# lucasgattas/ComfyUI-Egregora-Audio-Super-Resolution

Measured on AMD Instinct MI355X. Metric: audio-sec/sec (xRT) FlashSR 48kHz + Fat-Llama 800-iter at 1/2/4/8 MI355X, higher is better.
Workload: dtype f32(f16x2); 1 GPU; chain60: per GPU 60 s stereo 48 kHz; FlashSR (5.12 s chunks, hop 4.62 s, student_ldm 1-step + VAE + sr_vocoder, declared architecture, synthetic weights, chunk-sharded with one all-gather, WOLA) then Fat-Llama max_iterations=800 thr=0.6 normalize on autoscale off, threshold reading of the HEADLINE value: 'default' (SPEC.md section 3 default = absolute level on int16-scale samples, hard threshold, ; arch=gfx950:sramecc+:xnack-, chunks=13, rows_per_pass=32

## Files before the change

### comfyui-egregora-audio-super-resolution_amd/csrc/egr_flashsr.cpp

```cpp
#include <math.h>
#include <cmath>
#include <stdio.h>
#include <stdlib.h>
#include <string.h>

#include <atomic>
#include <chrono>
#include <map>
#include <memory>
#include <mutex>
#include <new>
#include <string>
#include <unordered_map>
#include <vector>

#include "egr_common.h"

extern "C" {
int egr_pack_weight(const float* src, float* dst, int layout, int K, int N, int Ci, int Co, int KH, int KW, void* stream);
int egr_phase_weights(const float* w_oihw, float* dst4, int Co, int Ci, void* stream);
int egr_winograd_pack_u(const float* w_oihw, float* dst, const double* G_dev, int np, int Co, int Ci, void* stream);
}

namespace {
// ... 964 lines not shown
            OKR(conv3(m, t, h, "vae.encoder.down." + std::to_string(lv) + ".downsample.conv", 2, 0, ACT_NONE, nullptr, 0));
            h = std::move(t);
        }
    }
    OKR(vae_res(m, t, h, "vae.encoder.mid.block_1")); h = std::move(t);
    OKR(vae_attn(m, t, h, "vae.encoder.mid.attn_1")); h = std::move(t);
    OKR(vae_res(m, t, h, "vae.encoder.mid.block_2")); h = std::move(t);
    OKR(groupnorm(m, t, h, "vae.encoder.norm_out", 1e-6f, true));
    OKR(conv3(m, h, t, "vae.encoder.conv_out"));
    Ten mom;
    OKR(conv1x1(m, mom, h, "vae.quant_conv"));
    const int64_t rows = mom.d[0] * mom.d[1] * mom.d[2];
    OKR(new_ten(m, z, {mom.d[0], mom.d[1], mom.d[2], c.z_ch}));
    EGR_HIP(hipMemcpy2DAsync(z.p, (size_t)c.z_ch * 4, mom.p, (size_t)2 * c.z_ch * 4, (size_t)c.z_ch * 4, (size_t)rows, hipMemcpyDeviceToDevice, m->st));
    return EGR_OK;
}

int vae_decode(M* m, Ten& y, const Ten& z) {
    const egr_flashsr_config& c = m->cfg;
    Ten h, t;
    m->next_out_ra = true;
    OKR(conv1x1(m, t, z, "vae.post_quant_conv"));
    OKR(conv3(m, h, t, "vae.decoder.conv_in"));
    OKR(vae_res(m, t, h, "vae.decoder.mid.block_1")); h = std::move(t);
    OKR(vae_attn(m, t, h, "vae.decoder.mid.attn_1")); h = std::move(t);
    OKR(vae_res(m, t, h, "vae.decoder.mid.block_2")); h = std::move(t);
    for (int lv = c.vae_levels - 1; lv >= 0; --lv) {
        for (int b = 0; b <= c.vae_res; ++b) {
            OKR(vae_res(m, t, h, "vae.decoder.up." + std::to_string(lv) + ".block." + std::to_string(b)));
            h = std::move(t);
        }
        if (lv != 0) {
            OKR(conv3(m, t, h, "vae.decoder.up." + std::to_string(lv) + ".upsample.conv", 1, 1));
            h = std::move(t);
        }
    }
    OKR(groupnorm(m, t, h, "vae.decoder.norm_out", 1e-6f, true));
    return conv3(m, y, t, "vae.decoder.conv_out");
}

int unet_block(M* m, Ten& y, const Ten& x, const std::string& base, bool has_attn) {
    const egr_flashsr_config& c = m->cfg;
    Ten h, sc, r;
    OKR(gn_conv3(m, h, x, base + ".res.in_norm", 1e-5f, base + ".res.in_conv", nullptr, m->ptr(base + ".res.in_conv.bias_t")));
    const float* scp = x.p;
    if (m->has(base + ".res.skip.weight")) { OKR(conv1x1(m, sc, x, base + ".res.skip")); scp = sc.p; }
    OKR(gn_conv3(m, r, h, base + ".res.out_norm", 1e-5f, base + ".res.out_conv", scp));
    h.release(); sc.release();
    if (!has_attn) { y = std::move(r); return EGR_OK; }
    const int B = (int)r.d[0], H = (int)r.d[1], W = (int)r.d[2], Cc = (int)r.d[3];
    const int T = H * W, heads = Cc / c.head_dim;
    Ten g0, t;
    OKR(groupnorm(m, g0, r, base + ".st.norm", 1e-6f, false));
    OKR(conv1x1(m, t, g0, base + ".st.proj_in"));
    g0.release();
    t.view({(int64_t)B * T, Cc});
    for (int a = 1; a <= 2; ++a) {
        const std::string an = base + ".st.attn" + std::to_string(a);
        Ten n_, q, k, v, o, t2;
        OKR(layernorm(m, n_, t, an + "_ln"));
        m->next_out_ra = true;
        OKR(linear(m, q, n_, an + ".to_q", nullptr, ACT_NONE, false));
        m->next_out_ra = true;
        OKR(linear(m, k, n_, an + ".to_k", nullptr, ACT_NONE, false));
        m->next_out_ra = true;
        OKR(linear(m, v, n_, an + ".to_v", nullptr, ACT_NONE, false));
        OKR(attention(m, o, q, k, v, B, T, Cc, heads));
        OKR(linear(m, t2, o, an + ".to_out", t.p));
        t = std::move(t2);
    }
    Ten ln, u, g, t3;
    OKR(layernorm(m, ln, t, base + ".st.ff_ln"));
    OKR(linear(m, u, ln, base + ".st.ff.geglu"));
    OKR(new_ten(m, g, {(int64_t)B * T, 4 * Cc}));
    {
        float* ra = nullptr;
        if (B == m->R) OKR(rs_for_output(m, g, &ra));
        if (ra) OKR(egr_geglu_ra(u.p, g.p, (int64_t)B * T, 4 * Cc, m->R, ra, m->st));
        else OKR(egr_geglu(u.p, g.p, (int64_t)B * T, 4 * Cc, m->st));
    }
    m->next_out_ra = true;
    OKR(linear(m, t3, g, base + ".st.ff.out", t.p));
    t3.view({B, H, W, Cc});
    m->next_out_ra = true;
    return conv1x1(m, y, t3, base + ".st.proj_out", r.p);
}

int unet(M* m, Ten& out, Ten&& x0) {
    std::vector<Ten> skips;
    Ten h = std::move(x0), t;
    for (size_t i = 0; i < m->blk_name.size(); ++i) {
        const std::string& name = m->blk_name[i];
        const std::string base = "unet." + name;
        const std::string part = name.substr(0, name.find('.'));
        const std::string kind = name.substr(name.rfind('.') + 1);
        if (kind == "conv_in") {
            OKR(conv3(m, t, h, base));
            Ten cp = t.alias();
            skips.push_back(std::move(t));
            h = std::move(cp);
        } else if (kind == "down") {
            m->next_out_ra = true;
            OKR(conv3(m, t, h, base + ".conv", 2, 0, ACT_NONE, nullptr, 1));
            Ten cp = t.alias();
            skips.push_back(std::move(t));
            h = std::move(cp);
        } else if (kind == "up") {
            OKR(conv3(m, t, h, base + ".conv", 1, 1));
            h = std::move(t);
        } else {
            if (part == "out") {
                Ten cat;
                OKR(concat(m, cat, h, skips.back()));
                skips.pop_back();
                h = std::move(cat);
            }
            OKR(unet_block(m, t, h, base, m->blk_attn[i] != 0));
            if (part == "in") {
                Ten cp = t.alias();
                skips.push_back(std::move(t));
                h = std::move(cp);
            } else {
                h = std::move(t);
            }
        }
    }
    OKR(groupnorm(m, t, h, "unet.out_norm", 1e-5f, true));
    return conv3(m, out, t, "unet.out_conv");
}

int amp(M* m, Ten& y, Ten&& h, int j) {
    const egr_flashsr_config& c = m->cfg;
    Ten acc;
    for (int ki = 0; ki < c.voc_n_kernels; ++ki) {
        const int k = c.voc_kernels[ki];
        Ten x;
        const Ten* cur = &h;
        for (int di = 0; di < c.voc_n_dils; ++di) {
            const int d = c.voc_dils[di];
            const std::string b = "voc.amp." + std::to_string(j) + "." + std::to_string(ki) + "." + std::to_string(di);
            Ten xt, xc, xs, xn;
            {
                const Wt* w1 = m->get(b + ".conv1.weight");
                const Wt* w2 = m->get(b + ".conv2.weight");
                const int Cc = (int)cur->d[2];
                if (m->fused_amp && m->h2 && m->h2_mode == 1 && w1 && w2 && w1->w2 && w2->w2 && Cc == 16 && w1->Cout == Cc && w2->Cout == Cc && (k & 1) &&
                    k <= 11 && d * (k - 1) / 2 <= 25 && c.aa_taps == 12 && cur->d[1] >= 16) {
                    OKR(new_ten(m, xn, {cur->d[0], cur->d[1], cur->d[2]}));
                    ProfScope ps(m);
                    OKR(egr_amp_unit_h2(cur->p, xn.p, (int)cur->d[0], (int)cur->d[1], Cc, k, d, m->ptr(b + ".alpha1"), m->ptr(b + ".beta1"), w1->w2, w1->w_scale,
                                        m->ptr(b + ".conv1.bias"), m->ptr(b + ".alpha2"), m->ptr(b + ".beta2"), w2->w2, w2->w_scale, m->ptr(b + ".conv2.bias"),
                                        m->filt, c.aa_taps, m->st));
                    const double fl = 2.0 * 2.0 * (double)cur->d[0] * cur->d[1] * Cc * Cc * k;
                    if (ps.on) ps.end(Cc == 16 ? "k_amp_unit<16>" : "k_amp_unit<32>", fl, b);
                    if (m->count_flops) m->flops += fl;
                    x = std::move(xn);
                    cur = &x;
                    continue;
                }
            }
            OKR(snake(m, xt, *cur, b + ".alpha1", b + ".beta1"));
            OKR(conv1d(m, xc, xt, b + ".conv1", k, 1, d, d * (k - 1) / 2));
            xt.release();
            OKR(snake(m, xs, xc, b + ".alpha2", b + ".beta2"));
            xc.release();
            OKR(conv1d(m, xn, xs, b + ".conv2", k, 1, 1, (k - 1) / 2, ACT_NONE, cur->p));
            x = std::move(xn);
            cur = &x;
        }
        if (ki == 0) {
            acc = std::move(x);
        } else if (ki + 1 < c.voc_n_kernels) {
            Ten s;
            OKR(eltwise(m, s, acc, x.p, EW_ADD));
            acc = std::move(s);
        } else {
            return eltwise(m, y, acc, x.p, EW_ADD_SCALE, 1.0f / c.voc_n_kernels, 0.f, true);
        }
    }
    return eltwise(m, y, acc, nullptr, EW_SCALE, 1.0f / c.voc_n_kernels, 0.f, true);
}

int vocoder(M* m, Ten& y, const Ten& mel_hat, const float* wave, int B) {
    const egr_flashsr_config& c = m->cfg;
    const int T = (int)mel_hat.d[1], Fm = (int)mel_hat.d[2];
    const int n = c.voc_n_rates;
    std::vector<Ten> feats(n);
    {
        Ten e0;
        e0.view({B, c.chunk, 1});
        e0.p = const_cast<float*>(wave);
        const Ten* e = &e0;
        for (int i = 0; i < n; ++i) {
            const int r = c.voc_rates[n - 1 - i];
            m->next_out_ra = i + 1 < n;
            OKR(conv1d(m, feats[i], *e, "voc.wave_enc." + std::to_string(i), 2 * r + 1, r, 1, r, ACT_LEAKY));
            e = &feats[i];
        }
    }
    Ten mh;
    mh.view({B, T, Fm});
    mh.p = mel_hat.p;
    Ten h;
    m->next_out_ra = true;
    OKR(conv1d(m, h, mh, "voc.conv_pre", 7, 1, 1, 3, ACT_NONE, feats[n - 1].p));
    feats[n - 1].release();
    for (int j = 0; j < n; ++j) {
        const int r = c.voc_rates[j];
        const int kt = up_kernel(r);
        const int Bc = (int)h.d[0], Lin = (int)h.d[1], Ci = (int)h.d[2];
        const Wt* wt = m->get("voc.ups." + std::to_string(j) + ".weight");
        const int Co = wt->Cout / kt;
        Ten Y, out, hx;
        hx.view({(int64_t)Bc * Lin, 1, 1, Ci});
        hx.p = h.p;
        hx.rs = h.rs;
        OKR(conv(m, Y, hx, "voc.ups." + std::to_string(j), Bc * Lin, 1, 1, Ci, 1, 1, kt * Co, 1, 1, 1, 1, 0, 0, 0, ACT_NONE, false, nullptr, nullptr, 0.f, wt));
        OKR(new_ten(m, out, {Bc, (int64_t)Lin * r, Co}));
        const float* add = (j <= n - 2) ? feats[n - 2 - j].p : nullptr;
        OKR(egr_col2im_convtr1d(Y.p, m->ptr("voc.ups." + std::to_string(j) + ".bias"), add, out.p, Bc, Lin, Lin * r, Co, kt, r, (kt - r) / 2, m->st));
        Y.release();
        if (j <= n - 2) feats[n - 2 - j].release();
        Ten nx;
        OKR(amp(m, nx, std::move(out), j));
        h = std::move(nx);
    }
    Ten s;
    OKR(snake(m, s, h, "voc.post.alpha", "voc.post.beta"));
    OKR(conv1d(m, y, s, "voc.conv_post", 7, 1, 1, 3, ACT_TANH));
    y.view({B, y.d[1]});
    return EGR_OK;
}

int copy_out(M* m, float* dst, const Ten& t) {
    if (!dst) return EGR_OK;
    EGR_HIP(hipMemcpyAsync(dst, t.p, (size_t)t.numel() * 4, hipMemcpyDeviceToDevice, m->st));
    return EGR_OK;
}

int forward(M* m, const float* x_in, const float* noise, int R, int lowpass_on, float* y_out, float* const* stages) {
    const egr_flashsr_config& c = m->cfg;
    const float* x = x_in;
    m->R = R;
    if (m->h2_mode == 1) {
        FsrCtx* cx = m->cx;
        size_t slices = (size_t)(2 * m->h2_nweights + 64);
        if (const char* e = getenv("EGR_FSR_RS_POOL_SLICES")) { const int v = atoi(e); if (v >= 1) slices = (size_t)v; }
        const size_t need = slices * (size_t)R * EGR_ROW_AMAX_STRIDE;
        if (!cx->rs_retired.empty()) {
            hipStreamSynchronize(m->st);
            for (unsigned* q : cx->rs_retired) hipFree(q);
            cx->rs_retired.clear();
        }
        if (cx->rs_cap < need) {
            if (cx->rs_pool) { hipStreamSynchronize(m->st); hipFree(cx->rs_pool); cx->rs_pool = nullptr; cx->rs_cap = 0; }
            if (hipMalloc((void**)&cx->rs_pool, need * sizeof(unsigned)) != hipSuccess) { set_error("hipMalloc(row maxima pool) failed"); return EGR_ERR_ALLOC; }
            cx->rs_cap = need;
        }
        EGR_HIP(hipMemsetAsync(cx->rs_pool, 0, cx->rs_cap * sizeof(unsigned), m->st));
        cx->rs_used = 0;
        if (cx->rs_ones_rows < R) {
            if (cx->rs_ones) { hipStreamSynchronize(m->st); hipFree(cx->rs_ones); cx->rs_ones = nullptr; }
            const size_t n = (size_t)R * EGR_ROW_AMAX_STRIDE;
            if (hipMalloc((void**)&cx->rs_ones, n * sizeof(unsigned)) != hipSuccess) { set_error("hipMalloc(row maxima constants) failed"); return EGR_ERR_ALLOC; }
            std::vector<unsigned> ones(n, 0x3f800000u);
            EGR_HIP(hipMemcpy(cx->rs_ones, ones.data(), n * sizeof(unsigned), hipMemcpyHostToDevice));
            cx->rs_ones_rows = R;
        }
    }
    static const int trace_lv = getenv("EGR_FSR_TRACE") ? atoi(getenv("EGR_FSR_TRACE")) : 0;
    const bool trace2 = trace_lv >= 2;
    const double t_fwd = now_ms();
    auto stage_mark = [&](const char* what) {
        if (trace_lv == 1) fprintf(stderr, "[egr_flashsr forward R=%d] %-10s enqueued at %8.1f ms\n", R, what, now_ms() - t_fwd);
        if (!trace2) return;
        const double t_host = now_ms() - t_fwd;
        hipStreamSynchronize(m->st);
        fprintf(stderr, "[egr_flashsr forward R=%d] %-10s enqueued at %8.1f ms, complete at %8.1f ms (arena hipMalloc so far %.1f ms)\n", R, what, t_host,
                now_ms() - t_fwd, 1e-3 * (double)g_arena_malloc_us.load());
    };
    Ten xl;
    if (lowpass_on) { OKR(lowpass(m, xl, x_in, R, c.chunk)); x = xl.p; }
    Ten mel, z_c, v, z0, mel_hat, y;
    OKR(log_mel(m, mel, x, R, c.chunk));
    stage_mark("log_mel");
    OKR(vae_encode(m, z_c, mel));
    stage_mark("vae_encode");
    {
        Ten nz, cat;
        nz.view({R, m->lat_h, m->lat_w, c.z_ch});
        nz.p = const_cast<float*>(noise);
        OKR(concat(m, cat, nz, z_c));
        OKR(unet(m, v, std::move(cat)));
        OKR(eltwise(m, z0, nz, v.p, EW_AXPBY, m->alpha, -m->sigma));
    }
    stage_mark("unet");
    OKR(vae_decode(m, mel_hat, z0));
    stage_mark("vae_decode");
    OKR(vocoder(m, y, mel_hat, x, R));
    stage_mark("vocoder");
    if (stages) {
        OKR(copy_out(m, stages[0], mel)); OKR(copy_out(m, stages[1], z_c)); OKR(copy_out(m, stages[2], v));
        OKR(copy_out(m, stages[3], z0)); OKR(copy_out(m, stages[4], mel_hat)); OKR(copy_out(m, stages[5], y));
    }
    const int64_t Ly = y.d[1];
    EGR_CHECK(Ly >= c.chunk, EGR_ERR_UNSUPPORTED, "FlashSR: vocoder output %lld shorter than the chunk %d", (long long)Ly, c.chunk);
    EGR_HIP(hipMemcpy2DAsync(y_out, (size_t)c.chunk * 4, y.p, (size_t)Ly * 4, (size_t)c.chunk * 4, (size_t)R, hipMemcpyDeviceToDevice, m->st));
// ... 456 lines not shown
```

### comfyui-egregora-audio-super-resolution_amd/csrc/egr_nn_amp.hip

```cpp
#include <stdlib.h>

#include "egr_conv.h"
#include "egr_s3_split.h"

namespace egr {

struct AmpP {
    const float* x; float* y;
    const float* alpha1; const float* beta1; const float* alpha2; const float* beta2; const float* filt;
    const uint4* w1; const uint4* w2;
    const float* bias1; const float* bias2;
    float inv_ws1, inv_ws2;
    int B, L, k, d;
};

typedef float f32x4 __attribute__((ext_vector_type(4)));

constexpr int AMP_SH = 5;
constexpr int AMP_MAXH1 = 25, AMP_MAXH2 = 5;

template <int C, int TL> struct AmpGeom {
    static constexpr int R0 = TL + 2 * (AMP_SH + AMP_MAXH1 + AMP_SH + AMP_MAXH2);
    static constexpr int XR = R0 + 16;
    static constexpr int RA = ((TL + 2 * (AMP_SH + AMP_MAXH2) + 15) / 16) * 16 + 2 * AMP_MAXH1 + 2;
    static constexpr int NCH = C / 8;
    static constexpr int LDS = XR * C * 4 + 2 * RA * NCH * 16;
};

template <int C, bool EDGE>
__device__ __forceinline__ void amp_snake_run(const float* __restrict__ S, int row0, int nrows, int l0, int c, int L, const float (&f)[12], const float (&f2)[12],
                                              float a_rev, float ib, float (&out)[16]) {
    constexpr int J = 16;
    float xw[J + 10];
    if constexpr (EDGE) {
#pragma unroll
        for (int i = 0; i < J + 10; ++i) {
            int src = l0 - 5 + i;
            src = src < 0 ? 0 : (src > L - 1 ? L - 1 : src);
            int r = src - row0;
            r = r < 0 ? 0 : (r > nrows - 1 ? nrows - 1 : r);
            xw[i] = S[r * C + c];
        }
    } else {
        const float* base = S + (l0 - 5 - row0) * C + c;
#pragma unroll
        for (int i = 0; i < J + 10; ++i) xw[i] = base[i * C];
    }
    float sv[2 * J + 10];
#pragma unroll
    for (int q = 0; q < 2 * J + 10; ++q) {
        float u = 0.f;
#pragma unroll
        for (int j = 0; j < 6; ++j) u += xw[5 + (q >> 1) - j] * f2[(q & 1) + 2 * j];
        const float sn = __builtin_amdgcn_sinf(__builtin_amdgcn_fractf(u * a_rev));
        sv[q] = fmaf(ib * sn, sn, u);
    }
    const int i0 = 2 * l0 - 5, L2 = 2 * L;
    if (EDGE && (i0 < 0 || i0 + 2 * J + 9 > L2 - 1)) {
        float s_first = 0.f, s_last = 0.f;
#pragma unroll
        for (int q = 0; q < 2 * J + 10; ++q) {
            if (i0 + q == 0) s_first = sv[q];
            if (i0 + q == L2 - 1) s_last = sv[q];
        }
#pragma unroll
        for (int q = 0; q < 2 * J + 10; ++q) {
            if (i0 + q < 0) sv[q] = s_first;
            if (i0 + q > L2 - 1) sv[q] = s_last;
        }
    }
#pragma unroll
    for (int jj = 0; jj < J; ++jj) {
        float acc = 0.f;
#pragma unroll
        for (int k = 0; k < 12; ++k) acc += f[k] * sv[2 * jj + k];
        out[jj] = acc;
    }
}

__device__ __forceinline__ float amp_wg_max(float m, float* slot) {
#pragma unroll
    for (int o = 32; o >= 1; o >>= 1) m = fmaxf(m, __shfl_xor(m, o));
    if ((threadIdx.x & 63) == 0) slot[threadIdx.x >> 6] = m;
    __syncthreads();
    const float r = fmaxf(fmaxf(slot[0], slot[1]), fmaxf(slot[2], slot[3]));
    __syncthreads();
    return r;
}

#ifndef AMP_LB16
#define AMP_LB16 2
#endif
#ifndef AMP_TL16
#define AMP_TL16 240
#endif
template <int C, int TL>
__global__ __launch_bounds__(256, C == 16 ? AMP_LB16 : 2) void k_amp_unit(AmpP p) {
    static_assert(C == 16, "K = 32 of v_mfma_f32_16x16x32_f16 = two taps of 16 channels (the 32-channel instantiation of round 5 -- half the "
                           "positions per tile -- lost to the four launches it replaced and was removed in round 6)");
    typedef AmpGeom<C, TL> G;
    constexpr int NCH = G::NCH;
    extern __shared__ __attribute__((aligned(16))) char smem[];
    float* XS = (float*)smem;
    uint4* AP = (uint4*)(smem + (size_t)G::XR * C * 4);
    __shared__ float red[4];
    const int tid = threadIdx.x, lane = tid & 63, wave = tid >> 6;
    const int b = blockIdx.y, t0 = blockIdx.x * TL;
    const int k = p.k, d = p.d, L = p.L;
    const int h2 = (k - 1) / 2, h1 = d * (k - 1) / 2;
    const int a2_row0 = t0 - h2, R3 = TL + 2 * h2;
    const int c1_row0 = a2_row0 - AMP_SH, R2 = R3 + 2 * AMP_SH;
    const int a1_row0 = c1_row0 - h1, R1 = R2 + 2 * h1;
    const int x_row0 = a1_row0 - AMP_SH, R0 = R1 + 2 * AMP_SH;
    const float* xb = p.x + (size_t)b * L * C;
    const bool interior = x_row0 >= 0 && x_row0 + R0 <= L;
    float f[12], f2[12];
#pragma unroll
    for (int i = 0; i < 12; ++i) { f[i] = p.filt[i]; f2[i] = 2.0f * f[i]; }
    float g_dn = 0.f, g_e = 0.f, g_o = 0.f;
#pragma unroll
    for (int i = 0; i < 12; ++i) { g_dn += fabsf(f[i]); if (i & 1) g_o += fabsf(f[i]); else g_e += fabsf(f[i]); }
    const float g_up = 2.0f * fmaxf(g_e, g_o);

    float vmax = 0.f;
    for (int e = tid; e < R0 * (C / 4); e += 256) {
        const int row = e / (C / 4), q = e - row * (C / 4);
        int l = x_row0 + row;
        l = l < 0 ? 0 : (l > L - 1 ? L - 1 : l);
        const float4 v = *(const float4*)(xb + (size_t)l * C + 4 * q);
        *(float4*)(XS + row * C + 4 * q) = v;
        vmax = fmaxf(vmax, fmaxf(fmaxf(fabsf(v.x), fabsf(v.y)), fmaxf(fabsf(v.z), fabsf(v.w))));
    }
    for (int e = R0 * (C / 4) + tid; e < G::XR * (C / 4); e += 256) *(float4*)(XS + e * 4) = make_float4(0.f, 0.f, 0.f, 0.f);
    const float xmax = amp_wg_max(vmax, red);

    auto snake_to_planes = [&](const float* S, int src_row0, int src_rows, int out_row0, int nrows_out, const float* alpha, const float* beta, float smax,
                               float& inv_scale) {
        float ibmax = 0.f;
#pragma unroll
        for (int c = 0; c < C; ++c) ibmax = fmaxf(ibmax, 1.0f / (__expf(beta[c]) + 1e-9f));
        const float bound = g_dn * (g_up * smax + ibmax);
        const unsigned bb = __float_as_uint(fmaxf(bound, 1e-30f));
        const float s = h2_row_scale(bb);
        inv_scale = h2_row_inv(bb);
        const int nruns = (nrows_out + 15) / 16;
        for (int it = tid; it < nruns * C; it += 256) {
            const int c = it % C, run = it / C;
            const int l0 = out_row0 + run * 16;
            const float a_rev = __expf(alpha[c]) * 0.15915494309189535f, ib = 1.0f / (__expf(beta[c]) + 1e-9f);
            float o[16];
            if (interior) amp_snake_run<C, false>(S, src_row0, src_rows, l0, c, L, f, f2, a_rev, ib, o);
            else amp_snake_run<C, true>(S, src_row0, src_rows, l0, c, L, f, f2, a_rev, ib, o);
            _Float16* P0 = (_Float16*)AP;
            _Float16* P1 = (_Float16*)(AP + (size_t)G::RA * NCH);
#pragma unroll
            for (int jj = 0; jj < 16; ++jj) {
                const int l = l0 + jj, r = run * 16 + jj;
                float v = (interior || (unsigned)l < (unsigned)L) ? o[jj] * s : 0.f;
                const _Float16 hi = (_Float16)v;
                const _Float16 lo = (_Float16)(v - (float)hi);
                if (r < G::RA) { P0[r * C + c] = hi; P1[r * C + c] = lo; }
            }
        }
    };

    const int m16 = lane & 15, kb = lane >> 4;
    constexpr int NH = C / 16, TPM = 32 / C, MAXB = (((TL + 2 * (AMP_SH + AMP_MAXH2) + 15) / 16) + 3) / 4;
    auto conv_planes = [&](const uint4* __restrict__ w, int dil, int nrows, auto&& emit) {
        const int nblk = (nrows + 15) / 16;
        f32x4 acc[MAXB][NH];
#pragma unroll
        for (int i = 0; i < MAXB; ++i)
#pragma unroll
            for (int nh = 0; nh < NH; ++nh) acc[i][nh] = f32x4{0.f, 0.f, 0.f, 0.f};
        const int nsteps = (k + TPM - 1) / TPM;
        for (int s = 0; s < nsteps; ++s) {
            const int tap = TPM == 2 ? 2 * s + (kb >> 1) : s;
            const bool tv = tap < k;
            const int tapc = tv ? tap : k - 1;
            uint4 bw[NH][2];
#pragma unroll
            for (int nh = 0; nh < NH; ++nh)
#pragma unroll
                for (int q = 0; q < 2; ++q) {
                    const size_t idx = C == 16 ? ((size_t)(tapc * 2 + q) * C + m16) * 2 + (kb & 1)
                                               : ((size_t)((tapc * 2 + (kb >> 1)) * 2 + q) * C + nh * 16 + m16) * 2 + (kb & 1);
                    const uint4 v = w[idx];
                    bw[nh][q] = tv ? v : make_uint4(0, 0, 0, 0);
                }
            const int chunk = C == 16 ? (kb & 1) : kb;
#pragma unroll
            for (int i = 0; i < MAXB; ++i) {
                const int rb = wave + 4 * i;
                if (rb < nblk) {
                    const int row = rb * 16 + m16 + tapc * dil;
                    const uint4 a0 = AP[(size_t)row * NCH + chunk];
                    const uint4 a1 = AP[((size_t)G::RA + row) * NCH + chunk];
#pragma unroll
                    for (int nh = 0; nh < NH; ++nh) {
                        acc[i][nh] = __builtin_amdgcn_mfma_f32_16x16x32_f16(as_hf(a1), as_hf(bw[nh][0]), acc[i][nh], 0, 0, 0);
                        acc[i][nh] = __builtin_amdgcn_mfma_f32_16x16x32_f16(as_hf(a0), as_hf(bw[nh][1]), acc[i][nh], 0, 0, 0);
                        acc[i][nh] = __builtin_amdgcn_mfma_f32_16x16x32_f16(as_hf(a0), as_hf(bw[nh][0]), acc[i][nh], 0, 0, 0);
                    }
                }
            }
        }
#pragma unroll
        for (int i = 0; i < MAXB; ++i) {
            const int rb = wave + 4 * i;
            if (rb < nblk) {
#pragma unroll
                for (int nh = 0; nh < NH; ++nh) emit(rb, nh, acc[i][nh]);
            }
        }
    };

    float inv_s1;
    snake_to_planes(XS, x_row0, R0, a1_row0, R1, p.alpha1, p.beta1, xmax, inv_s1);
    __syncthreads();

    float cmax_l = 0.f;
    {
        const float sc = inv_s1 * p.inv_ws1;
        conv_planes(p.w1, d, R2, [&](int rb, int nh, const f32x4& acc) {
            const int n = nh * 16 + m16;
            const float bias = p.bias1 ? p.bias1[n] : 0.f;
#pragma unroll
            for (int i = 0; i < 4; ++i) {
                const int r = rb * 16 + 4 * kb + i;
                const int l = c1_row0 + r;
                const float v = fmaf(acc[i], sc, bias);
                if (r < R2) {
                    XS[r * C + n] = v;
                    if ((unsigned)l < (unsigned)L) cmax_l = fmaxf(cmax_l, fabsf(v));
                }
            }
        });
    }
    const float cmax = amp_wg_max(cmax_l, red);

    float inv_s2;
    snake_to_planes(XS, c1_row0, R2, a2_row0, R3, p.alpha2, p.beta2, cmax, inv_s2);
    __syncthreads();

    {
        const float sc = inv_s2 * p.inv_ws2;
        float* yb = p.y + (size_t)b * L * C;
        conv_planes(p.w2, 1, TL, [&](int rb, int nh, const f32x4& acc) {
            const int n = nh * 16 + m16;
            const float bias = p.bias2 ? p.bias2[n] : 0.f;
#pragma unroll
            for (int i = 0; i < 4; ++i) {
                const int l = t0 + rb * 16 + 4 * kb + i;
                if (l < L) yb[(size_t)l * C + n] = fmaf(acc[i], sc, bias) + xb[(size_t)l * C + n];
            }
        });
    }
}

}

using namespace egr;

extern "C" int egr_amp_unit_h2(const float* x, float* y, int B, int L, int C, int k, int d, const float* alpha1, const float* beta1, const void* w1_h2,
                               float w1_scale, const float* bias1, const float* alpha2, const float* beta2, const void* w2_h2, float w2_scale,
                               const float* bias2, const float* filt, int aa_taps, void* stream) {
    EGR_CHECK(x && y && x != y && alpha1 && beta1 && alpha2 && beta2 && w1_h2 && w2_h2 && filt, EGR_ERR_ARG, "egr_amp_unit_h2: null argument");
    EGR_CHECK(B >= 1 && B <= 65535 && L >= 16 && w1_scale > 0.f && w2_scale > 0.f, EGR_ERR_ARG, "egr_amp_unit_h2: bad shape / scale");
    if (C != 16 || aa_taps != 12 || k < 1 || k > 11 || (k & 1) == 0 || d < 1 || d * (k - 1) / 2 > AMP_MAXH1 || (((uintptr_t)x) & 15) || (((uintptr_t)y) & 15)) {
        set_error("egr_amp_unit_h2: C = %d, k = %d, d = %d, %d FIR taps do not qualify (C = 16, odd k <= 11, d (k - 1) / 2 <= %d, 12 taps)", C, k, d, aa_taps, AMP_MAXH1);
        return EGR_ERR_UNSUPPORTED;
    }
    AmpP p;
    p.x = x; p.y = y; p.alpha1 = alpha1; p.beta1 = beta1; p.alpha2 = alpha2; p.beta2 = beta2; p.filt = filt;
    p.w1 = (const uint4*)w1_h2; p.w2 = (const uint4*)w2_h2; p.bias1 = bias1; p.bias2 = bias2;
    p.inv_ws1 = 1.0f / w1_scale; p.inv_ws2 = 1.0f / w2_scale;
    p.B = B; p.L = L; p.k = k; p.d = d;
    {
        constexpr int TL = AMP_TL16;
        constexpr size_t lds = (size_t)AmpGeom<16, TL>::LDS;
        hipLaunchKernelGGL((k_amp_unit<16, TL>), dim3((unsigned)((L + TL - 1) / TL), (unsigned)B), dim3(256), lds, (hipStream_t)stream, p);
    }
    EGR_HIP(hipGetLastError());
    return EGR_OK;
}
```

Baseline: 279.0 audio-sec/sec.

## Make fused AMP unit kernel persistent with async LDS prefetch of next tile

Replaces the one-tile-per-workgroup AMP residual-unit kernel with a persistent kernel sized to occupancy. Each workgroup loops over a contiguous range of (batch, tile) items. The next tile's input is loaded straight into LDS with global_load_lds while the current tile's second convolution runs. Conv weights are staged once in LDS, LDS sizing now depends on the actual k and d instead of the worst case, and barriers are lighter. The cost is added complexity and hand-written inline asm with manual vmcnt waits, which could be fragile. The input buffer is reused for the prefetch, so the residual is read from global memory before the emit step.

Measured after the change: 280.3 audio-sec/sec (median of 6 runs). No clear change (+0.5%).

```diff
diff --git a/comfyui-egregora-audio-super-resolution_amd/csrc/egr_flashsr.cpp b/comfyui-egregora-audio-super-resolution_amd/csrc/egr_flashsr.cpp
--- a/comfyui-egregora-audio-super-resolution_amd/csrc/egr_flashsr.cpp
+++ b/comfyui-egregora-audio-super-resolution_amd/csrc/egr_flashsr.cpp
@@ -1140,7 +1140,7 @@
                                         m->ptr(b + ".conv1.bias"), m->ptr(b + ".alpha2"), m->ptr(b + ".beta2"), w2->w2, w2->w_scale, m->ptr(b + ".conv2.bias"),
                                         m->filt, c.aa_taps, m->st));
                     const double fl = 2.0 * 2.0 * (double)cur->d[0] * cur->d[1] * Cc * Cc * k;
-                    if (ps.on) ps.end(Cc == 16 ? "k_amp_unit<16>" : "k_amp_unit<32>", fl, b);
+                    if (ps.on) ps.end("k_amp_unit_persist<16>", fl, b);
                     if (m->count_flops) m->flops += fl;
                     x = std::move(xn);
                     cur = &x;
diff --git a/comfyui-egregora-audio-super-resolution_amd/csrc/egr_nn_amp.hip b/comfyui-egregora-audio-super-resolution_amd/csrc/egr_nn_amp.hip
--- a/comfyui-egregora-audio-super-resolution_amd/csrc/egr_nn_amp.hip
+++ b/comfyui-egregora-audio-super-resolution_amd/csrc/egr_nn_amp.hip
@@ -1,4 +1,7 @@
 #include <stdlib.h>
+
+#include <mutex>
+#include <vector>
 
 #include "egr_conv.h"
 #include "egr_s3_split.h"
@@ -19,14 +22,6 @@
 constexpr int AMP_SH = 5;
 constexpr int AMP_MAXH1 = 25, AMP_MAXH2 = 5;
 
-template <int C, int TL> struct AmpGeom {
-    static constexpr int R0 = TL + 2 * (AMP_SH + AMP_MAXH1 + AMP_SH + AMP_MAXH2);
-    static constexpr int XR = R0 + 16;
-    static constexpr int RA = ((TL + 2 * (AMP_SH + AMP_MAXH2) + 15) / 16) * 16 + 2 * AMP_MAXH1 + 2;
-    static constexpr int NCH = C / 8;
-    static constexpr int LDS = XR * C * 4 + 2 * RA * NCH * 16;
-};
-
 template <int C, bool EDGE>
 __device__ __forceinline__ void amp_snake_run(const float* __restrict__ S, int row0, int nrows, int l0, int c, int L, const float (&f)[12], const float (&f2)[12],
                                               float a_rev, float ib, float (&out)[16]) {
@@ -78,42 +73,79 @@
     }
 }
 
+__device__ __forceinline__ void amp_barrier() {
+    asm volatile("s_waitcnt lgkmcnt(0)" ::: "memory");
+    __builtin_amdgcn_s_barrier();
+    asm volatile("" ::: "memory");
+}
+
+__device__ __forceinline__ void amp_glds16(const void* src, const void* lds_wave_base) {
+    const unsigned m = __builtin_amdgcn_readfirstlane((unsigned)(size_t)(const __attribute__((address_space(3))) char*)lds_wave_base);
+    unsigned keep;
+    asm volatile("s_mov_b32 %0, m0\n\ts_mov_b32 m0, %2\n\ts_nop 0\n\tglobal_load_lds_dwordx4 %1, off\n\ts_mov_b32 m0, %0" : "=&s"(keep) : "v"(src), "s"(m) : "memory");
+}
+
 __device__ __forceinline__ float amp_wg_max(float m, float* slot) {
 #pragma unroll
     for (int o = 32; o >= 1; o >>= 1) m = fmaxf(m, __shfl_xor(m, o));
     if ((threadIdx.x & 63) == 0) slot[threadIdx.x >> 6] = m;
-    __syncthreads();
-    const float r = fmaxf(fmaxf(slot[0], slot[1]), fmaxf(slot[2], slot[3]));
-    __syncthreads();
-    return r;
-}
-
-#ifndef AMP_LB16
-#define AMP_LB16 2
+    amp_barrier();
+    return fmaxf(fmaxf(slot[0], slot[1]), fmaxf(slot[2], slot[3]));
+}
+
+template <int TL> struct AmpRows {
+    int R0, XR, RA;
+    __host__ __device__ AmpRows(int k, int d) {
+        const int h2 = (k - 1) / 2, h1 = d * (k - 1) / 2;
+        R0 = TL + 2 * (AMP_SH + h1 + AMP_SH + h2);
+        XR = R0 + 16;
+        RA = ((TL + 2 * (AMP_SH + h2) + 15) / 16) * 16 + 2 * h1 + 2;
+    }
+    __host__ __device__ size_t lds(int k, bool w2l) const { return (size_t)XR * 64 + (size_t)2 * RA * 32 + (size_t)(w2l ? 2 : 1) * k * 1024 + 32; }
+};
+
+#ifndef AMP_WGS
+#define AMP_WGS 3
 #endif
-#ifndef AMP_TL16
-#define AMP_TL16 240
-#endif
-template <int C, int TL>
-__global__ __launch_bounds__(256, C == 16 ? AMP_LB16 : 2) void k_amp_unit(AmpP p) {
-    static_assert(C == 16, "K = 32 of v_mfma_f32_16x16x32_f16 = two taps of 16 channels (the 32-channel instantiation of round 5 -- half the "
-                           "positions per tile -- lost to the four launches it replaced and was removed in round 6)");
-    typedef AmpGeom<C, TL> G;
-    constexpr int NCH = G::NCH;
+template <int TL, bool W2L>
+__global__ __launch_bounds__(256, AMP_WGS) void k_amp_unit_persist(AmpP p) {
+    constexpr int C = 16, NCH = 2;
     extern __shared__ __attribute__((aligned(16))) char smem[];
-    float* XS = (float*)smem;
-    uint4* AP = (uint4*)(smem + (size_t)G::XR * C * 4);
-    __shared__ float red[4];
     const int tid = threadIdx.x, lane = tid & 63, wave = tid >> 6;
-    const int b = blockIdx.y, t0 = blockIdx.x * TL;
     const int k = p.k, d = p.d, L = p.L;
     const int h2 = (k - 1) / 2, h1 = d * (k - 1) / 2;
-    const int a2_row0 = t0 - h2, R3 = TL + 2 * h2;
-    const int c1_row0 = a2_row0 - AMP_SH, R2 = R3 + 2 * AMP_SH;
-    const int a1_row0 = c1_row0 - h1, R1 = R2 + 2 * h1;
-    const int x_row0 = a1_row0 - AMP_SH, R0 = R1 + 2 * AMP_SH;
-    const float* xb = p.x + (size_t)b * L * C;
-    const bool interior = x_row0 >= 0 && x_row0 + R0 <= L;
+    const AmpRows<TL> G(k, d);
+    const int R3 = TL + 2 * h2, R2 = R3 + 2 * AMP_SH, R1 = R2 + 2 * h1, R0 = G.R0, RA = G.RA;
+    const int xbytes = G.XR * C * 4;
+    uint4* AP = (uint4*)(smem + xbytes);
+    uint4* W1 = AP + 2 * RA * NCH;
+    uint4* W2 = W1 + k * 64;
+    float* red = (float*)(W2 + (W2L ? k * 64 : 0));
+    const int ntiles = (L + TL - 1) / TL;
+    const long long total = (long long)p.B * ntiles;
+    const long long it0 = blockIdx.x * total / gridDim.x, it1 = (blockIdx.x + 1) * total / gridDim.x;
+    if (it0 >= it1) return;
+
+    auto dma_tile = [&](long long item) {
+        const int b = (int)(item / ntiles), t = (int)(item - (long long)b * ntiles);
+        const int x_row0 = t * TL - (h2 + AMP_SH + h1 + AMP_SH);
+        const char* xb = (const char*)(p.x + (size_t)b * L * C);
+        char* dst = smem;
+        int e0 = tid;
+        asm volatile("" : "+v"(e0));
+        for (int e = e0; e < R0 * 4; e += 256) {
+            int l = x_row0 + (e >> 2);
+            l = l < 0 ? 0 : (l > L - 1 ? L - 1 : l);
+            amp_glds16(xb + (size_t)l * (C * 4) + (e & 3) * 16, dst + (e & ~63) * 16);
+        }
+    };
+    dma_tile(it0);
+
+    for (int e = tid; e < k * 64; e += 256) {
+        W1[e] = p.w1[e];
+        if (W2L) W2[e] = p.w2[e];
+    }
+    if (tid < 64) *(float4*)(smem + (R0 * 4 + tid) * 16) = make_float4(0.f, 0.f, 0.f, 0.f);
     float f[12], f2[12];
 #pragma unroll
     for (int i = 0; i < 12; ++i) { f[i] = p.filt[i]; f2[i] = 2.0f * f[i]; }
@@ -121,146 +153,191 @@
 #pragma unroll
     for (int i = 0; i < 12; ++i) { g_dn += fabsf(f[i]); if (i & 1) g_o += fabsf(f[i]); else g_e += fabsf(f[i]); }
     const float g_up = 2.0f * fmaxf(g_e, g_o);
-
-    float vmax = 0.f;
-    for (int e = tid; e < R0 * (C / 4); e += 256) {
-        const int row = e / (C / 4), q = e - row * (C / 4);
-        int l = x_row0 + row;
-        l = l < 0 ? 0 : (l > L - 1 ? L - 1 : l);
-        const float4 v = *(const float4*)(xb + (size_t)l * C + 4 * q);
-        *(float4*)(XS + row * C + 4 * q) = v;
-        vmax = fmaxf(vmax, fmaxf(fmaxf(fabsf(v.x), fabsf(v.y)), fmaxf(fabsf(v.z), fabsf(v.w))));
-    }
-    for (int e = R0 * (C / 4) + tid; e < G::XR * (C / 4); e += 256) *(float4*)(XS + e * 4) = make_float4(0.f, 0.f, 0.f, 0.f);
-    const float xmax = amp_wg_max(vmax, red);
-
-    auto snake_to_planes = [&](const float* S, int src_row0, int src_rows, int out_row0, int nrows_out, const float* alpha, const float* beta, float smax,
-                               float& inv_scale) {
-        float ibmax = 0.f;
-#pragma unroll
-        for (int c = 0; c < C; ++c) ibmax = fmaxf(ibmax, 1.0f / (__expf(beta[c]) + 1e-9f));
-        const float bound = g_dn * (g_up * smax + ibmax);
-        const unsigned bb = __float_as_uint(fmaxf(bound, 1e-30f));
-        const float s = h2_row_scale(bb);
-        inv_scale = h2_row_inv(bb);
-        const int nruns = (nrows_out + 15) / 16;
-        for (int it = tid; it < nruns * C; it += 256) {
-            const int c = it % C, run = it / C;
-            const int l0 = out_row0 + run * 16;
-            const float a_rev = __expf(alpha[c]) * 0.15915494309189535f, ib = 1.0f / (__expf(beta[c]) + 1e-9f);
-            float o[16];
-            if (interior) amp_snake_run<C, false>(S, src_row0, src_rows, l0, c, L, f, f2, a_rev, ib, o);
-            else amp_snake_run<C, true>(S, src_row0, src_rows, l0, c, L, f, f2, a_rev, ib, o);
-            _Float16* P0 = (_Float16*)AP;
-            _Float16* P1 = (_Float16*)(AP + (size_t)G::RA * NCH);
-#pragma unroll
-            for (int jj = 0; jj < 16; ++jj) {
-                const int l = l0 + jj, r = run * 16 + jj;
-                float v = (interior || (unsigned)l < (unsigned)L) ? o[jj] * s : 0.f;
-                const _Float16 hi = (_Float16)v;
-                const _Float16 lo = (_Float16)(v - (float)hi);
-                if (r < G::RA) { P0[r * C + c] = hi; P1[r * C + c] = lo; }
+    float ibmax1 = 0.f, ibmax2 = 0.f;
+#pragma unroll
+    for (int c = 0; c < C; ++c) {
+        ibmax1 = fmaxf(ibmax1, 1.0f / (__expf(p.beta1[c]) + 1e-9f));
+        ibmax2 = fmaxf(ibmax2, 1.0f / (__expf(p.beta2[c]) + 1e-9f));
+    }
+    const int sc_ = tid & (C - 1);
+    const float a_rev1 = __expf(p.alpha1[sc_]) * 0.15915494309189535f, ib1 = 1.0f / (__expf(p.beta1[sc_]) + 1e-9f);
+    const float a_rev2 = __expf(p.alpha2[sc_]) * 0.15915494309189535f, ib2 = 1.0f / (__expf(p.beta2[sc_]) + 1e-9f);
+    const int m16 = lane & 15, kb = lane >> 4;
+    const float bias1 = p.bias1 ? p.bias1[m16] : 0.f, bias2 = p.bias2 ? p.bias2[m16] : 0.f;
+    asm volatile("s_waitcnt vmcnt(0)" ::: "memory");
+    amp_barrier();
+
+    for (long long it = it0; it < it1; ++it) {
+        const int b = (int)(it / ntiles), t0 = (int)(it - (long long)b * ntiles) * TL;
+        const int a2_row0 = t0 - h2;
+        const int c1_row0 = a2_row0 - AMP_SH;
+        const int a1_row0 = c1_row0 - h1;
+        const int x_row0 = a1_row0 - AMP_SH;
+        const bool interior = x_row0 >= 0 && x_row0 + R0 <= L;
+        float* XS = (float*)smem;
+
+        float vmax = 0.f;
+        for (int e = tid; e < R0 * (C / 4); e += 256) {
+            const float4 v = *(const float4*)(XS + e * 4);
+            vmax = fmaxf(vmax, fmaxf(fmaxf(fabsf(v.x), fabsf(v.y)), fmaxf(fabsf(v.z), fabsf(v.w))));
+        }
+        const float xmax = amp_wg_max(vmax, red);
+
+        auto snake_to_planes = [&](const float* S, int src_row0, int src_rows, int out_row0, int nrows_out, float a_rev, float ib, float ibmax, float smax,
+                                   float& inv_scale) {
+            const float bound = g_dn * (g_up * smax + ibmax);
+            const unsigned bb = __float_as_uint(fmaxf(bound, 1e-30f));
+            const float s = h2_row_scale(bb);
+            inv_scale = h2_row_inv(bb);
+            const int nruns = (nrows_out + 15) / 16;
+            for (int it2 = tid; it2 < nruns * C; it2 += 256) {
+                const int c = it2 % C, run = it2 / C;
+                const int l0 = out_row0 + run * 16;
+                float o[16];
+                if (interior) amp_snake_run<C, false>(S, src_row0, src_rows, l0, c, L, f, f2, a_rev, ib, o);
+                else amp_snake_run<C, true>(S, src_row0, src_rows, l0, c, L, f, f2, a_rev, ib, o);
+                _Float16* P0 = (_Float16*)AP;
+                _Float16* P1 = (_Float16*)(AP + (size_t)RA * NCH);
+#pragma unroll
+                for (int jj = 0; jj < 16; ++jj) {
+                    const int l = l0 + jj, r = run * 16 + jj;
+                    float v = (interior || (unsigned)l < (unsigned)L) ? o[jj] * s : 0.f;
+                    const _Float16 hi = (_Float16)v;
+                    const _Float16 lo = (_Float16)(v - (float)hi);
+                    if (r < RA) { P0[r * C + c] = hi; P1[r * C + c] = lo; }
+                }
             }
-        }
-    };
-
-    const int m16 = lane & 15, kb = lane >> 4;
-    constexpr int NH = C / 16, TPM = 32 / C, MAXB = (((TL + 2 * (AMP_SH + AMP_MAXH2) + 15) / 16) + 3) / 4;
-    auto conv_planes = [&](const uint4* __restrict__ w, int dil, int nrows, auto&& emit) {
-        const int nblk = (nrows + 15) / 16;
-        f32x4 acc[MAXB][NH];
-#pragma unroll
-        for (int i = 0; i < MAXB; ++i)
-#pragma unroll
-            for (int nh = 0; nh < NH; ++nh) acc[i][nh] = f32x4{0.f, 0.f, 0.f, 0.f};
-        const int nsteps = (k + TPM - 1) / TPM;
-        for (int s = 0; s < nsteps; ++s) {
-            const int tap = TPM == 2 ? 2 * s + (kb >> 1) : s;
-            const bool tv = tap < k;
-            const int tapc = tv ? tap : k - 1;
-            uint4 bw[NH][2];
-#pragma unroll
-            for (int nh = 0; nh < NH; ++nh)
+        };
+
+        constexpr int MAXB = (((TL + 2 * (AMP_SH + AMP_MAXH2) + 15) / 16) + 3) / 4;
+        auto conv_planes = [&](const uint4* w, int dil, int nrows, auto&& before_emit, auto&& emit) {
+            const int nblk = (nrows + 15) / 16;
+            f32x4 acc[MAXB];
+#pragma unroll
+            for (int i = 0; i < MAXB; ++i) acc[i] = f32x4{0.f, 0.f, 0.f, 0.f};
+            const int nsteps = (k + 1) / 2;
+            for (int s = 0; s < nsteps; ++s) {
+                const int tap = 2 * s + (kb >> 1);
+                const bool tv = tap < k;
+                const int tapc = tv ? tap : k - 1;
+                uint4 bw[2];
 #pragma unroll
                 for (int q = 0; q < 2; ++q) {
-                    const size_t idx = C == 16 ? ((size_t)(tapc * 2 + q) * C + m16) * 2 + (kb & 1)
-                                               : ((size_t)((tapc * 2 + (kb >> 1)) * 2 + q) * C + nh * 16 + m16) * 2 + (kb & 1);
-                    const uint4 v = w[idx];
-                    bw[nh][q] = tv ? v : make_uint4(0, 0, 0, 0);
-                }
-            const int chunk = C == 16 ? (kb & 1) : kb;
+                    const uint4 v = w[((tapc * 2 + q) * C + m16) * 2 + (kb & 1)];
+                    bw[q] = tv ? v : make_uint4(0, 0, 0, 0);
+                }
+                const int chunk = kb & 1;
+#pragma unroll
+                for (int i = 0; i < MAXB; ++i) {
+                    const int rb = wave + 4 * i;
+                    if (rb < nblk) {
+                        const int row = rb * 16 + m16 + tapc * dil;
+                        const uint4 a0 = AP[row * NCH + chunk];
+                        const uint4 a1 = AP[(RA + row) * NCH + chunk];
+                        acc[i] = __builtin_amdgcn_mfma_f32_16x16x32_f16(as_hf(a1), as_hf(bw[0]), acc[i], 0, 0, 0);
+                        acc[i] = __builtin_amdgcn_mfma_f32_16x16x32_f16(as_hf(a0), as_hf(bw[1]), acc[i], 0, 0, 0);
+                        acc[i] = __builtin_amdgcn_mfma_f32_16x16x32_f16(as_hf(a0), as_hf(bw[0]), acc[i], 0, 0, 0);
+                    }
+                }
+            }
+            before_emit();
 #pragma unroll
             for (int i = 0; i < MAXB; ++i) {
                 const int rb = wave + 4 * i;
-                if (rb < nblk) {
-                    const int row = rb * 16 + m16 + tapc * dil;
-                    const uint4 a0 = AP[(size_t)row * NCH + chunk];
-                    const uint4 a1 = AP[((size_t)G::RA + row) * NCH + chunk];
-#pragma unroll
-                    for (int nh = 0; nh < NH; ++nh) {
-                        acc[i][nh] = __builtin_amdgcn_mfma_f32_16x16x32_f16(as_hf(a1), as_hf(bw[nh][0]), acc[i][nh], 0, 0, 0);
-                        acc[i][nh] = __builtin_amdgcn_mfma_f32_16x16x32_f16(as_hf(a0), as_hf(bw[nh][1]), acc[i][nh], 0, 0, 0);
-                        acc[i][nh] = __builtin_amdgcn_mfma_f32_16x16x32_f16(as_hf(a0), as_hf(bw[nh][0]), acc[i][nh], 0, 0, 0);
+                if (rb < nblk) emit(i, rb, acc[i]);
+            }
+        };
+
+        float inv_s1;
+        snake_to_planes(XS, x_row0, R0, a1_row0, R1, a_rev1, ib1, ibmax1, xmax, inv_s1);
+        amp_barrier();
+
+        float cmax_l = 0.f;
+        {
+            const float sc = inv_s1 * p.inv_ws1;
+            conv_planes(W1, d, R2, [] {}, [&](int, int rb, const f32x4& acc) {
+#pragma unroll
+                for (int i = 0; i < 4; ++i) {
+                    const int r = rb * 16 + 4 * kb + i;
+                    const int l = c1_row0 + r;
+                    const float v = fmaf(acc[i], sc, bias1);
+                    if (r < R2) {
+                        XS[r * C + m16] = v;
+                        if ((unsigned)l < (unsigned)L) cmax_l = fmaxf(cmax_l, fabsf(v));
                     }
                 }
-            }
-        }
-#pragma unroll
-        for (int i = 0; i < MAXB; ++i) {
-            const int rb = wave + 4 * i;
-            if (rb < nblk) {
-#pragma unroll
-                for (int nh = 0; nh < NH; ++nh) emit(rb, nh, acc[i][nh]);
-            }
-        }
-    };
-
-    float inv_s1;
-    snake_to_planes(XS, x_row0, R0, a1_row0, R1, p.alpha1, p.beta1, xmax, inv_s1);
-    __syncthreads();
-
-    float cmax_l = 0.f;
-    {
-        const float sc = inv_s1 * p.inv_ws1;
-        conv_planes(p.w1, d, R2, [&](int rb, int nh, const f32x4& acc) {
-            const int n = nh * 16 + m16;
-            const float bias = p.bias1 ? p.bias1[n] : 0.f;
-#pragma unroll
-            for (int i = 0; i < 4; ++i) {
-                const int r = rb * 16 + 4 * kb + i;
-                const int l = c1_row0 + r;
-                const float v = fmaf(acc[i], sc, bias);
-                if (r < R2) {
-                    XS[r * C + n] = v;
-                    if ((unsigned)l < (unsigned)L) cmax_l = fmaxf(cmax_l, fabsf(v));
-                }
-            }
-        });
-    }
-    const float cmax = amp_wg_max(cmax_l, red);
-
-    float inv_s2;
-    snake_to_planes(XS, c1_row0, R2, a2_row0, R3, p.alpha2, p.beta2, cmax, inv_s2);
-    __syncthreads();
-
-    {
-        const float sc = inv_s2 * p.inv_ws2;
+            });
+        }
+        const float cmax = amp_wg_max(cmax_l, red + 4);
+
+        float inv_s2;
+        snake_to_planes(XS, c1_row0, R2, a2_row0, R3, a_rev2, ib2, ibmax2, cmax, inv_s2);
+        amp_barrier();
+
+        const float* xb = p.x + (size_t)b * L * C;
         float* yb = p.y + (size_t)b * L * C;
-        conv_planes(p.w2, 1, TL, [&](int rb, int nh, const f32x4& acc) {
-            const int n = nh * 16 + m16;
-            const float bias = p.bias2 ? p.bias2[n] : 0.f;
-#pragma unroll
-            for (int i = 0; i < 4; ++i) {
-                const int l = t0 + rb * 16 + 4 * kb + i;
-                if (l < L) yb[(size_t)l * C + n] = fmaf(acc[i], sc, bias) + xb[(size_t)l * C + n];
-            }
-        });
+        {
+            if (it + 1 < it1) dma_tile(it + 1);
+            const float sc = inv_s2 * p.inv_ws2;
+            float xres[MAXB][4];
+            auto conv2 = [&](const uint4* w2) {
+            conv_planes(w2, 1, TL, [&] {
+#pragma unroll
+                for (int j = 0; j < MAXB; ++j)
+#pragma unroll
+                    for (int i = 0; i < 4; ++i) {
+                        const int l = t0 + (wave + 4 * j) * 16 + 4 * kb + i;
+                        xres[j][i] = xb[(size_t)(l < L ? l : L - 1) * C + m16];
+                    }
+            }, [&](int j, int, const f32x4& acc) {
+#pragma unroll
+                for (int i = 0; i < 4; ++i) xres[j][i] = fmaf(acc[i], sc, bias2) + xres[j][i];
+            });
+            };
+            if constexpr (W2L) conv2(W2);
+            else conv2(p.w2);
+#pragma unroll
+            for (int j = 0; j < MAXB; ++j)
+#pragma unroll
+                for (int i = 0; i < 4; ++i) {
+                    const int l = t0 + (wave + 4 * j) * 16 + 4 * kb + i;
+                    if (wave + 4 * j < TL / 16 && l < L) yb[(size_t)l * C + m16] = xres[j][i];
+                }
+        }
+        if (interior) asm volatile("s_waitcnt vmcnt(12)" ::: "memory");
+        else asm volatile("s_waitcnt vmcnt(0)" ::: "memory");
+        amp_barrier();
     }
 }
 
 }
 
 using namespace egr;
+
+static hipError_t amp_residency(bool w2l, size_t lds, int* per_cu, int* cus) {
+    struct Entry { int dev; size_t lds; int per_cu, cus; };
+    static std::mutex mu;
+    static std::vector<Entry> seen;
+    int dev = 0;
+    hipError_t e = hipGetDevice(&dev);
+    if (e != hipSuccess) return e;
+    std::lock_guard<std::mutex> lock(mu);
+    for (const Entry& s : seen)
+        if (s.dev == dev && s.lds == lds) { *per_cu = s.per_cu; *cus = s.cus; return hipSuccess; }
+    Entry n{dev, lds, 0, 0};
+    if ((e = hipDeviceGetAttribute(&n.cus, hipDeviceAttributeMultiprocessorCount, dev)) != hipSuccess) return e;
+    int lds_max = 0;
+    if ((e = hipDeviceGetAttribute(&lds_max, hipDeviceAttributeMaxSharedMemoryPerBlock, dev)) != hipSuccess) return e;
+    if (lds == 0) n.per_cu = lds_max;
+    else if (lds <= (size_t)lds_max) {
+        const void* kern = w2l ? (const void*)k_amp_unit_persist<240, true> : (const void*)k_amp_unit_persist<240, false>;
+        if ((e = hipFuncSetAttribute(kern, hipFuncAttributeMaxDynamicSharedMemorySize, lds_max)) != hipSuccess) return e;
+        if ((e = hipOccupancyMaxActiveBlocksPerMultiprocessor(&n.per_cu, kern, 256, lds)) != hipSuccess) return e;
+    }
+    seen.push_back(n);
+    *per_cu = n.per_cu; *cus = n.cus;
+    return hipSuccess;
+}
 
 extern "C" int egr_amp_unit_h2(const float* x, float* y, int B, int L, int C, int k, int d, const float* alpha1, const float* beta1, const void* w1_h2,
                                float w1_scale, const float* bias1, const float* alpha2, const float* beta2, const void* w2_h2, float w2_scale,
@@ -276,11 +353,15 @@
     p.w1 = (const uint4*)w1_h2; p.w2 = (const uint4*)w2_h2; p.bias1 = bias1; p.bias2 = bias2;
     p.inv_ws1 = 1.0f / w1_scale; p.inv_ws2 = 1.0f / w2_scale;
     p.B = B; p.L = L; p.k = k; p.d = d;
-    {
-        constexpr int TL = AMP_TL16;
-        constexpr size_t lds = (size_t)AmpGeom<16, TL>::LDS;
-        hipLaunchKernelGGL((k_amp_unit<16, TL>), dim3((unsigned)((L + TL - 1) / TL), (unsigned)B), dim3(256), lds, (hipStream_t)stream, p);
-    }
+    constexpr int TL = 240;
+    int lds_cu = 0, per_cu = 0, cus = 0;
+    EGR_HIP(amp_residency(true, 0, &lds_cu, &cus));
+    const bool w2l = AMP_WGS * AmpRows<TL>(k, d).lds(k, true) <= (size_t)lds_cu;
+    const size_t lds = AmpRows<TL>(k, d).lds(k, w2l);
+    EGR_HIP(amp_residency(w2l, lds, &per_cu, &cus));
+    EGR_CHECK(per_cu >= 1 && cus >= 1, EGR_ERR_HIP, "egr_amp_unit_h2: %zu bytes of LDS per workgroup do not fit a compute unit", lds);
+    if (w2l) hipLaunchKernelGGL((k_amp_unit_persist<TL, true>), dim3((unsigned)(per_cu * cus)), dim3(256), lds, (hipStream_t)stream, p);
+    else hipLaunchKernelGGL((k_amp_unit_persist<TL, false>), dim3((unsigned)(per_cu * cus)), dim3(256), lds, (hipStream_t)stream, p);
     EGR_HIP(hipGetLastError());
     return EGR_OK;
 }
```
